# shoeffner/ann3depth

Hardware: AMD Instinct MI355X
Metric: images/sec (640x480->55x74 MSDN train step) (higher is better)
Workload: dtype f32

## Files before the change

### ann3depth_amd/csrc/fewch.hip

```cpp
#include <algorithm>

#include "a3d_internal.h"
#include "igemm.h"

namespace a3d {

enum { FEW_SRC_DZ = 0, FEW_SRC_POOLED = 1, FEW_SRC_POOLED_BF16 = 2 };
constexpr int kFewRows = 6;

struct FewchParams {
  const float* x;
  const void* dz;
  const void* pooled;
  const uint8_t* argmax;
  float* slabs;
  int n, h, w, c, R, S, stride, ho, wo, N, M, Mp, NP;
  int ldz, ld_arg;
  int rows_per_img, rows_total, splits, mgroups;
  int xpitch, rowlen, kpairs, wo_pad;
  int xvec4, dvec4;
};

typedef float f32x16 __attribute__((ext_vector_type(16)));

// ... 182 lines not shown
    A3D_STAMP(s3);
    const float* ap = xs + a_off;
    const float* bp = dzs + lh * NP + li;
    const int groups = p.kpairs >> 2;
    const bool more = row + 1 < row_hi;
    float a[2][4], b[2][4][TN];
    auto read = [&](int buf) {
#pragma unroll
      for (int u = 0; u < 4; ++u) {
        a[buf][u] = ap[u * a_step];
#pragma unroll
        for (int t = 0; t < TN; ++t) b[buf][u][t] = bp[u * 2 * NP + t * 32];
      }
      ap += 4 * a_step;
      bp += 8 * NP;
    };
    auto mul = [&](int buf) {
#pragma unroll
      for (int u = 0; u < 4; ++u)
#pragma unroll
        for (int t = 0; t < TN; ++t) acc[t] = __builtin_amdgcn_mfma_f32_32x32x2f32(a[buf][u], b[buf][u][t], acc[t], 0, 0, 0);
    };
    int g = 0;
    if (groups >= 2) {
      read(0);
      read(1);
      mul(0);
      if (more) fetch(row + 1);
      if (groups > 2) read(0);
      mul(1);
      for (g = 2; g + 2 <= groups; g += 2) {
        read(1);
        mul(0);
        if (g + 2 < groups) read(0);
        mul(1);
      }
      if (g < groups) mul(0);
      g = groups;
    } else if (more) {
      fetch(row + 1);
    }
    for (int kp = g * 4; kp < p.kpairs; ++kp) {
      const float av1 = ap[0];
#pragma unroll
      for (int t = 0; t < TN; ++t) acc[t] = __builtin_amdgcn_mfma_f32_32x32x2f32(av1, bp[t * 32], acc[t], 0, 0, 0);
      ap += a_step;
      bp += 2 * NP;
    }
#ifdef A3D_STAMPS
    A3D_STAMP(s4);
    d_ld += s_ld - s_mid; d_xw += s_mid - s1; d_bar1 += s1 - s0; d_commit += s2 - s1; d_bar2 += s3 - s2; d_mfma += s4 - s3;
#endif
  }
#ifdef A3D_STAMPS
  if (lane == 0 && blockIdx.x < 1024) {
    unsigned long long t_end;
    A3D_STAMP(t_end);
    unsigned long long* o = g_fewch_stamps + ((size_t)blockIdx.x * 4 + wv) * 8;
    o[0] = d_bar1; o[1] = d_commit; o[2] = d_bar2; o[3] = d_mfma; o[4] = (unsigned long long)(row_hi - row_lo); o[5] = d_xw; o[6] = t_end;
    o[7] = d_ld;
  }
  unsigned long long t_end2 = 0;
  A3D_STAMP(t_end2);
#endif
  float* slab = p.slabs + ((size_t)split * p.Mp + mg * 128 + wv * 32) * NP;
#pragma unroll
  for (int t = 0; t < TN; ++t)
#pragma unroll
    for (int g = 0; g < 4; ++g)
#pragma unroll
      for (int i = 0; i < 4; ++i) slab[(size_t)(8 * g + 4 * lh + i) * NP + t * 32 + li] = acc[t][4 * g + i];
#ifdef A3D_STAMPS
  asm volatile("s_waitcnt vmcnt(0)" ::: "memory");
  unsigned long long t_exit = 0;
  A3D_STAMP(t_exit);
  if (lane == 0 && blockIdx.x < 1024) {
    unsigned long long* o = g_fewch_stamps + ((size_t)blockIdx.x * 4 + wv) * 8;
    o[5] = t_exit - t_end2;
    o[6] = t_end2 - t_entry;
  }
#endif
}

__global__ __launch_bounds__(256) void fewch_reduce_kernel(const float* __restrict__ slabs, int splits, int Mp, int NP, int M, int N,
                                                           float* __restrict__ dw, float* __restrict__ db) {
  const int idx = blockIdx.x * 256 + threadIdx.x;
  if (idx >= (M + 1) * N) return;
  const int m = idx / N, n = idx - m * N;
  const float* s = slabs + (size_t)m * NP + n;
  const size_t pitch = (size_t)Mp * NP;
  float a0 = 0.f;
  int k = 0;
  for (; k + 8 <= splits; k += 8) {
    float v[8];
#pragma unroll
    for (int u = 0; u < 8; ++u) v[u] = s[(size_t)(k + u) * pitch];
#pragma unroll
    for (int u = 0; u < 8; ++u) a0 += v[u];
  }
  for (; k < splits; ++k) a0 += s[(size_t)k * pitch];
  if (m < M) dw[(size_t)m * N + n] = a0;
  else if (db) db[n] = a0;
}

struct FewchShape {
  int M, Mp, mgroups, TN, NP, rows_per_img, rows_total, splits, xpitch, wo_pad, kpairs;
  size_t lds;
};

static FewchShape fewch_shape(const a3d_conv_desc* d, bool pooled) {
  FewchShape s;
  s.M = d->r * d->s * d->c;
  s.mgroups = (s.M + 1 + 127) / 128;
  s.Mp = s.mgroups * 128;
  s.TN = (d->k + 31) / 32;
  s.NP = s.TN * 32;
  s.rows_per_img = pooled ? (d->ho / 2) * 2 : d->ho;
  s.rows_total = d->n * s.rows_per_img;
  s.wo_pad = (d->wo + 1) / 2 * 2;
  s.kpairs = s.wo_pad / 2;
  const int reach = (s.wo_pad - 1) * d->stride * d->c + d->s * d->c;
  s.xpitch = (std::max(d->w * d->c, reach) + 3) / 4 * 4;
  s.splits = std::max(1, std::min(s.rows_total / 4, tune_int("A3D_FEWCH_BLOCKS", 512) / s.mgroups));
  s.lds = (size_t)((kFewRows + 2) * s.xpitch + s.wo_pad * s.NP + 256 * 4 + s.NP + 4) * 4;
  return s;
}

bool fewch_bwdf_applicable(const a3d_conv_desc* d, bool pooled) {
  if (d->precision != A3D_PREC_F32 || d->c > 4 || d->pad_t || d->pad_l || d->ldx != d->c) return false;
  if (d->k < 33 || d->k > 96) return false;
  if (d->s * d->c < 27) return false;
  if ((d->ho - 1) * d->stride + d->r > d->h || (d->wo - 1) * d->stride + d->s > d->w) return false;
  if (pooled && (d->ho < 2 || d->wo < 2)) return false;
  if ((d->w * d->c) % 4 != 0) return false;
  if ((double)d->n * d->h * d->w * d->c * 4.0 >= 2147483647.0) return false;
  const FewchShape s = fewch_shape(d, pooled);
  if (s.rows_total < 1 || s.lds > 78 * 1024) return false;
  if (kFewRows * (d->w * d->c / 4) > kPX * 256) return false;
  if ((pooled ? d->wo / 2 : d->wo) * ((d->k + 3) / 4) > (pooled ? kPDPooled : kPDPlain) * 256) return false;
  return true;
}

bool fewch_extents_ok(const a3d_conv_desc* d, bool pooled, int ldz, int esz, int ld_arg) {
  const double pixels = pooled ? (double)d->n * (d->ho / 2) * (d->wo / 2) : (double)d->n * d->ho * d->wo;
  return pixels * ldz * esz < 2147483647.0 && (!pooled || pixels * ld_arg < 2147483647.0);
}

size_t fewch_bwdf_ws_bytes(const a3d_conv_desc* d, bool pooled) {
  const FewchShape s = fewch_shape(d, pooled);
  return (size_t)s.splits * s.Mp * s.NP * 4 + 16;
}

template <int TN, int SRC, bool VEC, int STEP>
static void fewch_launch4(const FewchParams& p, int blocks, size_t lds, hipStream_t st) {
  (void)hipFuncSetAttribute(reinterpret_cast<const void*>(&fewch_bwdf_kernel<TN, SRC, VEC, STEP>), hipFuncAttributeMaxDynamicSharedMemorySize,
                            80 * 1024);
  hipLaunchKernelGGL((fewch_bwdf_kernel<TN, SRC, VEC, STEP>), dim3(blocks), dim3(256), lds, st, p);
}
template <int TN, int SRC, bool VEC>
static void fewch_launch3(const FewchParams& p, int blocks, size_t lds, hipStream_t st) {
  const int step = p.stride * p.c;
  if (TN == 3 && step == 12) return fewch_launch4<TN, SRC, VEC, TN == 3 ? 12 : 0>(p, blocks, lds, st);
  if (TN == 2 && step == 6) return fewch_launch4<TN, SRC, VEC, TN == 2 ? 6 : 0>(p, blocks, lds, st);
  if (TN == 2 && step == 3) return fewch_launch4<TN, SRC, VEC, TN == 2 ? 3 : 0>(p, blocks, lds, st);
  fewch_launch4<TN, SRC, VEC, 0>(p, blocks, lds, st);
}
template <int TN>
static void fewch_launch(int src, const FewchParams& p, int blocks, size_t lds, hipStream_t st) {
  if (src == FEW_SRC_DZ) p.dvec4 ? fewch_launch3<TN, FEW_SRC_DZ, true>(p, blocks, lds, st) : fewch_launch3<TN, FEW_SRC_DZ, false>(p, blocks, lds, st);
  else if (src == FEW_SRC_POOLED) p.dvec4 ? fewch_launch3<TN, FEW_SRC_POOLED, true>(p, blocks, lds, st) : fewch_launch3<TN, FEW_SRC_POOLED, false>(p, blocks, lds, st);
  else p.dvec4 ? fewch_launch3<TN, FEW_SRC_POOLED_BF16, true>(p, blocks, lds, st) : fewch_launch3<TN, FEW_SRC_POOLED_BF16, false>(p, blocks, lds, st);
}

int fewch_bwd_filter(const a3d_conv_desc* d, const float* x, int src, const void* dz, int ldz, const void* pooled_act,
                     const uint8_t* argmax, int ld_arg, float* dw, float* db, void* ws, hipStream_t st) {
  const bool pooled = src != FEW_SRC_DZ;
  const FewchShape s = fewch_shape(d, pooled);
  FewchParams p{};
  p.x = x; p.dz = dz; p.pooled = pooled_act; p.argmax = argmax;
  p.slabs = reinterpret_cast<float*>((reinterpret_cast<uintptr_t>(ws) + 15) & ~(uintptr_t)15);
  p.n = d->n; p.h = d->h; p.w = d->w; p.c = d->c; p.R = d->r; p.S = d->s; p.stride = d->stride; p.ho = d->ho; p.wo = d->wo;
  p.N = d->k; p.M = s.M; p.Mp = s.Mp; p.NP = s.NP; p.ldz = ldz; p.ld_arg = ld_arg;
  p.rows_per_img = s.rows_per_img; p.rows_total = s.rows_total; p.splits = s.splits; p.mgroups = s.mgroups;
  p.xpitch = s.xpitch; p.rowlen = d->w * d->c; p.kpairs = s.kpairs; p.wo_pad = s.wo_pad;
  p.xvec4 = p.rowlen % 4 == 0 && (reinterpret_cast<uintptr_t>(x) & 15) == 0;
  p.dvec4 = pooled ? (d->k % 4 == 0 && ld_arg % 4 == 0 && (reinterpret_cast<uintptr_t>(argmax) & 3) == 0)
                   : (d->k % 4 == 0 && ldz % 4 == 0 && (reinterpret_cast<uintptr_t>(dz) & 15) == 0);
  const int blocks = s.splits * s.mgroups;
  clear_stale_error();
  if (s.TN == 3) fewch_launch<3>(src, p, blocks, s.lds, st);
  else fewch_launch<2>(src, p, blocks, s.lds, st);
  int rc = check_launch("fewch_bwd_filter");
  if (rc != A3D_OK) return rc;
  return fewch_reduce_launch(p.slabs, s.splits, s.Mp, s.NP, s.M, d->k, dw, db, st);
}

#ifdef A3D_STAMPS
extern "C" int a3d_debug_fewch_stamps(unsigned long long* out, size_t bytes) {
  (void)hipDeviceSynchronize();
  return (int)hipMemcpyFromSymbol(out, HIP_SYMBOL(g_fewch_stamps), std::min(bytes, sizeof(g_fewch_stamps)));
}
#endif

int fewch_reduce_launch(const float* slabs, int splits, int Mp, int NP, int M, int N, float* dw, float* db, hipStream_t st) {
  const int outs = (M + 1) * N;
  clear_stale_error();
  hipLaunchKernelGGL(fewch_reduce_kernel, dim3((outs + 255) / 256), dim3(256), 0, st, slabs, splits, Mp, NP, M, N, dw, db);
  return check_launch("fewch_reduce");
}

}
```

### ann3depth_amd/csrc/igemm.h

```cpp
#pragma once
#include <hip/hip_runtime.h>
#include <stdint.h>

#include <type_traits>

#include "igemm_plan.h"

namespace a3d {

#ifdef A3D_STAMPS
#define A3D_STAMP(var)                                                                         \
  do {                                                                                         \
    __builtin_amdgcn_sched_barrier(0);                                                         \
    unsigned long long t_;                                                                     \
    asm volatile("s_memtime %0\n\ts_waitcnt lgkmcnt(0)" : "=s"(t_)::"memory");                 \
    __builtin_amdgcn_sched_barrier(0);                                                         \
    var = t_;                                                                                  \
  } while (0)
#define A3D_RTSTAMP(var)                                                                       \
  do {                                                                                         \
    __builtin_amdgcn_sched_barrier(0);                                                         \
    unsigned long long t_;                                                                     \
    asm volatile("s_memrealtime %0\n\ts_waitcnt lgkmcnt(0)" : "=s"(t_)::"memory");             \
    __builtin_amdgcn_sched_barrier(0);                                                         \
// ... 333 lines not shown
  return (uint32_t)(((unsigned long long)b * total) / nblk);
}

template <int TM, int TN>
__device__ __forceinline__ void slab_store(float* slab, const f32x16 (&acc)[TM][TN], int wave, int lane) {
#pragma unroll
  for (int a = 0; a < TM; ++a)
#pragma unroll
    for (int b = 0; b < TN; ++b)
#pragma unroll
      for (int q = 0; q < 4; ++q) {
        const f32x4 v = {acc[a][b][4 * q], acc[a][b][4 * q + 1], acc[a][b][4 * q + 2], acc[a][b][4 * q + 3]};
        *reinterpret_cast<f32x4*>(slab + ((((size_t)(wave * TM + a) * TN + b) * 4 + q) * 64 + lane) * 4) = v;
      }
}
template <int TM, int TN>
__device__ __forceinline__ void slab_add(const float* slab, f32x16 (&acc)[TM][TN], int wave, int lane) {
#pragma unroll
  for (int a = 0; a < TM; ++a)
#pragma unroll
    for (int b = 0; b < TN; ++b)
#pragma unroll
      for (int q = 0; q < 4; ++q) {
        const f32x4 v = *reinterpret_cast<const f32x4*>(slab + ((((size_t)(wave * TM + a) * TN + b) * 4 + q) * 64 + lane) * 4);
        acc[a][b][4 * q] += v[0]; acc[a][b][4 * q + 1] += v[1]; acc[a][b][4 * q + 2] += v[2]; acc[a][b][4 * q + 3] += v[3];
      }
}

template <int MODE>
__device__ __forceinline__ void store_quad(const IgemmParams& p, const f32x4 q, int row0, int col, float* Cout, int ldc,
                                           bool partial) {
  if (col >= p.N) return;
  float v[4];
  size_t o[4];
  bool ok[4];
  const bool remap = !partial && MODE == MODE_BWD_D;
#pragma unroll
  for (int i = 0; i < 4; ++i) {
    const int row = row0 + i;
    v[i] = q[i];
    ok[i] = row < p.M;
    o[i] = (remap ? remap_row(ok[i] ? row : 0, p.sub_step, p.sub_ph, p.sub_pw, p.outW, p.outHW, p.div_phw, p.div_pw) : (size_t)row) *
               ldc + col;
  }
  if (!partial) {
    if (MODE == MODE_FWD) {
      const float bias = p.bias ? p.bias[col] : 0.f;
#pragma unroll
      for (int i = 0; i < 4; ++i) v[i] += bias;
      if (p.act == EPI_RELU) {
#pragma unroll
        for (int i = 0; i < 4; ++i) v[i] = fmaxf(v[i], 0.f);
      } else if (p.act == EPI_SIGMOID) {
#pragma unroll
        for (int i = 0; i < 4; ++i) v[i] = 1.f / (1.f + __expf(-v[i]));
      }
      if (p.keep) {
        uint8_t k[4];
#pragma unroll
        for (int i = 0; i < 4; ++i) k[i] = ok[i] ? p.keep[(size_t)(row0 + i) * p.N + col] : (uint8_t)0;
#pragma unroll
        for (int i = 0; i < 4; ++i) v[i] = k[i] ? v[i] * p.mask_scale : 0.f;
      }
    } else if (MODE == MODE_BWD_D) {
      if (p.mask) {
        float y[4];
#pragma unroll
        for (int i = 0; i < 4; ++i) y[i] = ok[i] ? p.mask[o[i]] : 0.f;
#pragma unroll
        for (int i = 0; i < 4; ++i) v[i] = apply_act_grad(v[i], y[i], p.mask_act, p.mask_scale);
      }
    }
  }
  if (p.c16 && !partial) {
#pragma unroll
    for (int i = 0; i < 4; ++i)
      if (ok[i]) reinterpret_cast<__bf16*>(Cout)[o[i]] = (__bf16)v[i];
  } else {
#pragma unroll
    for (int i = 0; i < 4; ++i)
      if (ok[i]) Cout[o[i]] = v[i];
  }
}
template <int MODE, int TM, int TN, int WM, int WN>
__device__ __forceinline__ void store_tile(const IgemmParams& p, const f32x16 (&acc)[TM][TN], int m0, int n0, int wm,
                                           int wn, int li, int lh, float* Cout, int ldc, bool partial) {
#pragma unroll
  for (int a = 0; a < TM; ++a)
#pragma unroll
    for (int b = 0; b < TN; ++b)
#pragma unroll
      for (int q = 0; q < 4; ++q) {
        const f32x4 v = {acc[a][b][4 * q], acc[a][b][4 * q + 1], acc[a][b][4 * q + 2], acc[a][b][4 * q + 3]};
        store_quad<MODE>(p, v, m0 + wm * WM + a * 32 + 8 * q + 4 * lh, n0 + wn * WN + b * 32 + li, Cout, ldc, partial);
      }
}

__device__ __forceinline__ __amdgpu_buffer_rsrc_t epi_rsrc(const void* base, size_t byte_off, uint32_t bytes) {
  const unsigned long long a = reinterpret_cast<unsigned long long>(base) + byte_off;
  const uint32_t lo = __builtin_amdgcn_readfirstlane((uint32_t)a), hi = __builtin_amdgcn_readfirstlane((uint32_t)(a >> 32));
  return __builtin_amdgcn_make_buffer_rsrc(reinterpret_cast<void*>(((unsigned long long)hi << 32) | lo), 0,
                                           (int)__builtin_amdgcn_readfirstlane(bytes), 0x00020000);
}
template <int MODE>
__device__ __forceinline__ bool epi_buf_ok(const IgemmParams& p, int ldc, bool partial) {
  if (ldc >= (1 << 21)) return false;
  if (partial) return true;
  if (MODE == MODE_BWD_D && p.sub_step > 1) return false;
  if (MODE == MODE_FWD && p.keep) return false;
  return true;
}
template <int MODE, int BM, int TM, int TN, int WM, int WN, bool MASK16, bool FASTEXP = true>
__device__ __forceinline__ void store_tile_buf(const IgemmParams& p, f32x16 (&acc)[TM][TN], int m0, int n0, int wm, int wn,
                                               int li, int lh, float* Cout, int ldc, bool partial, bool c16) {
  int rows_left = p.M - m0;
  rows_left = rows_left < 0 ? 0 : (rows_left > BM ? BM : rows_left);
  const uint32_t row_el = (uint32_t)((wm * WM + 4 * lh) * ldc);
  uint32_t elb[TN];
  bool okb[TN];
#pragma unroll
  for (int b = 0; b < TN; ++b) {
    const int col = n0 + wn * WN + b * 32 + li;
    okb[b] = col < p.N;
    elb[b] = row_el + (uint32_t)col;
  }
  auto row_off = [&](int a, int e) -> uint32_t { return (uint32_t)((a * 32 + 8 * (e >> 2) + (e & 3)) * ldc); };
  if (!partial) {
    if (MODE == MODE_FWD) {
      float bias[TN];
#pragma unroll
      for (int b = 0; b < TN; ++b) bias[b] = (p.bias && okb[b]) ? p.bias[n0 + wn * WN + b * 32 + li] : 0.f;
#pragma unroll
      for (int a = 0; a < TM; ++a)
#pragma unroll
        for (int b = 0; b < TN; ++b)
#pragma unroll
          for (int e = 0; e < 16; ++e) acc[a][b][e] += bias[b];
      if (p.act == EPI_RELU) {
#pragma unroll
        for (int a = 0; a < TM; ++a)
#pragma unroll
          for (int b = 0; b < TN; ++b)
#pragma unroll
            for (int e = 0; e < 16; ++e) acc[a][b][e] = fmaxf(acc[a][b][e], 0.f);
      } else if (p.act == EPI_SIGMOID) {
#pragma unroll
        for (int a = 0; a < TM; ++a)
#pragma unroll
          for (int b = 0; b < TN; ++b)
#pragma unroll
            for (int e = 0; e < 16; ++e) acc[a][b][e] = 1.f / (1.f + (FASTEXP ? __expf(-acc[a][b][e]) : expf(-acc[a][b][e])));
      }
    } else if (MODE == MODE_BWD_D) {
      if (p.mask) {
        constexpr uint32_t MSZ = MASK16 ? 2u : 4u;
        const __amdgpu_buffer_rsrc_t rsM = epi_rsrc(p.mask, (size_t)m0 * ldc * MSZ, (uint32_t)(rows_left * ldc) * MSZ);
#pragma unroll
        for (int a = 0; a < TM; ++a)
#pragma unroll
          for (int b = 0; b < TN; ++b) {
            const uint32_t vb = okb[b] ? elb[b] * MSZ : kOOB;
            float y[16];
#pragma unroll
            for (int e = 0; e < 16; ++e) {
              if constexpr (MASK16)
                y[e] = (float)__builtin_bit_cast(
// ... 488 lines not shown
        }
      }
    } else {
#pragma unroll
    for (int u = 0; u < BK / 8; ++u) {
      f32x4 af[TM], bf[TN];
      const int kk = 8 * u + 4 * lh;
#pragma unroll
      for (int a = 0; a < TM; ++a) {
        const int row = (wm * Cfg::WM + a * 32 + li) ^ (Cfg::A_SWZ ? 32 * lh : 0);
        if (MODE == MODE_BWD_F) {
#pragma unroll
          for (int j = 0; j < 4; ++j) af[a][j] = Ac[(kk + j) * Cfg::A_LD + row];
        } else {
          af[a] = *reinterpret_cast<const f32x4*>(Ac + row * Cfg::A_LD + kk);
        }
      }
#pragma unroll
      for (int b = 0; b < TN; ++b) {
        const int col = (wn * Cfg::WN + b * 32 + li) ^ (Cfg::B_SWZ ? 32 * lh : 0);
        if (MODE == MODE_BWD_D) {
          bf[b] = *reinterpret_cast<const f32x4*>(Bc + col * Cfg::B_LD + kk);
        } else {
#pragma unroll
          for (int j = 0; j < 4; ++j) bf[b][j] = Bc[(kk + j) * Cfg::B_LD + col];
        }
      }
      if (u == BK / 8 - 1) {
        A3D_STAMP(s2);
        if (more) store_tiles(cur ^ 1);
        A3D_STAMP(s3);
      }
#pragma unroll
      for (int j = 0; j < 4; ++j)
#pragma unroll
        for (int a = 0; a < TM; ++a)
#pragma unroll
          for (int b = 0; b < TN; ++b)
            acc[a][b] = __builtin_amdgcn_mfma_f32_32x32x2f32(af[a][j], bf[b][j], acc[a][b], 0, 0, 0);
    }
    }
    A3D_STAMP(s4);
    __syncthreads();
    A3D_STAMP(s5);
#ifdef A3D_STAMPS
    d01 += s1 - s0; d12 += s2 - s1; d23 += s3 - s2; d34 += s4 - s3; d45 += s5 - s4;
#endif
  };
  for (int it = 0; it < nkt; it += 2) {
    tile_body(it, std::integral_constant<int, 0>{});
    if (it + 1 < nkt) tile_body(it + 1, std::integral_constant<int, 1>{});
  }
  };
  if constexpr (MODE == MODE_BWD_F) {
    k_loop(std::false_type{});
  } else {
    if (p.uni) k_loop(std::true_type{});
    else k_loop(std::false_type{});
  }
#ifdef A3D_STAMPS
  A3D_STAMP(tend);
  A3D_RTSTAMP(rtend);
  if (p.stamps && lane == 0) {
    unsigned long long* o = p.stamps + ((size_t)bid_in * NWAVES + wave) * 16;
    o[0] = d01; o[1] = d12; o[2] = d23; o[3] = d34; o[4] = d45; o[5] = tend - tbeg; o[6] = (unsigned long long)nkt; o[7] = tp1 - t_entry; o[15] = tp2 - tp1;
    o[8] = tbeg - t_entry; o[9] = t_entry; o[10] = tend; o[12] = rtend - rtbeg; o[13] = rtbeg; o[14] = rtend;
  }
#define A3D_STAMP_EXIT()                                                                                   \
  do {                                                                                                     \
    unsigned long long t_exit_;                                                                            \
    A3D_STAMP(t_exit_);                                                                                    \
    if (p.stamps && lane == 0) p.stamps[((size_t)bid_in * NWAVES + wave) * 16 + 11] = t_exit_;              \
  } while (0)
#else
#define A3D_STAMP_EXIT() do { } while (0)
#endif

  igemm_epilogue<MODE, BM, BN, TM, TN, Cfg::WM, Cfg::WN>(p, acc, split, bid, seg, kt_begin, kt_end, nk_total, do_bias, bsum, tid, wave, lane,
                                                          m0, n0, wm, wn);
  }
  A3D_STAMP_EXIT();
}

template <int MODE, int BM, int BN, int WAVES_M, int NWAVES>
__global__ __launch_bounds__(256) void igemm_fixup_kernel(const IgemmParams p, const uint32_t nblk) {
  constexpr int WAVES_N = NWAVES / WAVES_M, WM = BM / WAVES_M, WN = BN / WAVES_N, TM = WM / 32, TN = WN / 32;
  constexpr int UNITS = NWAVES * TM * TN * 4;
  constexpr int MAXC = 1024;
  __shared__ uint32_t slots[MAXC];
  __shared__ uint32_t nslots;
  const int lane = threadIdx.x & 63;
  const int unit = (int)blockIdx.y * 4 + (int)(threadIdx.x >> 6);
  const uint32_t tile = blockIdx.x;
  const uint32_t nk = p.div_nk.d, tiles = (uint32_t)(p.tiles_m * p.tiles_n);
  if (threadIdx.x == 0) {
    uint32_t n = 0;
    const uint32_t total = tiles * nk, t0 = tile * nk, t1 = t0 + nk - 1;
    uint32_t jf = (uint32_t)(((unsigned long long)t0 * nblk) / total), jl = (uint32_t)(((unsigned long long)t1 * nblk) / total);
    while (jf + 1 < nblk && sk_first(jf + 1, nblk, total) <= t0) ++jf;
    while (jl + 1 < nblk && sk_first(jl + 1, nblk, total) <= t1) ++jl;
    for (uint32_t b = jf; b <= jl; ++b) {
      const uint32_t f = sk_first(b, nblk, total);
      if (f == sk_first(b + 1, nblk, total)) continue;
      if (n < MAXC) slots[n] = 2 * b + (f / nk == tile ? 0u : 1u);
      ++n;
    }
    nslots = n < MAXC ? n : MAXC;
  }
  __syncthreads();
  const uint32_t n = nslots;
  if (n <= 1) return;
  const int tile_m = (int)tile / p.tiles_n, tile_n = (int)tile - tile_m * p.tiles_n;
  if (unit < UNITS) {
    const size_t uoff = ((size_t)unit * 64 + lane) * 4;
    f32x4 s = {0.f, 0.f, 0.f, 0.f};
    auto slab_of = [&](uint32_t i) -> f32x4 {
      return *reinterpret_cast<const f32x4*>(p.sk_ws + (size_t)slots[i] * (size_t)(BM * BN) + uoff);
    };
    uint32_t i = 0;
    for (; i + 8 <= n; i += 8) {
      f32x4 v[8];
#pragma unroll
      for (int u = 0; u < 8; ++u) v[u] = slab_of(i + u);
#pragma unroll
      for (int u = 0; u < 8; ++u) s += v[u];
    }
    if (i + 4 <= n) {
      const f32x4 v0 = slab_of(i), v1 = slab_of(i + 1), v2 = slab_of(i + 2), v3 = slab_of(i + 3);
      s += v0; s += v1; s += v2; s += v3;
      i += 4;
    }
    for (; i < n; ++i) s += slab_of(i);
    const int q = unit & 3, ab = unit >> 2, bb = ab % TN, a = (ab / TN) % TM, wave = ab / (TN * TM);
    const int wm = wave / WAVES_N, wn = wave % WAVES_N, li = lane & 31, lh = lane >> 5;
    store_quad<MODE>(p, s, tile_m * BM + wm * WM + a * 32 + 8 * q + 4 * lh, tile_n * BN + wn * WN + bb * 32 + li, p.C,
                     p.ldc, false);
  }
  if (MODE == MODE_BWD_F && p.dbias != nullptr && tile_m == 0 && blockIdx.y == 0 && (int)threadIdx.x < BN) {
    static_assert(BN <= 256, "bias sums by the first 256 threads");
    float bsum = 0.f;
    for (uint32_t i = 0; i < n; ++i) bsum += p.sk_bias[(size_t)slots[i] * BN + threadIdx.x];
    if (tile_n * BN + (int)threadIdx.x < p.N) p.dbias[tile_n * BN + threadIdx.x] = bsum;
  }
}

template <int MODE, int BM, int BN, int WAVES_M, int NWAVES, int BKT, int AVEC, int BVEC>
__global__ __launch_bounds__(64 * NWAVES, (BKT == 16 ? 3 : 2) * NWAVES / 4) void igemm_kernel(const IgemmParams p) {
  igemm_body<MODE, BM, BN, WAVES_M, NWAVES, BKT, AVEC, BVEC>(p, gridDim.x, blockIdx.x);
}

struct IgemmMulti {
  IgemmParams p[4];
};
template <int MODE, int BM, int BN, int WAVES_M, int NWAVES, int BKT, int AVEC, int BVEC>
__global__ __launch_bounds__(64 * NWAVES, (BKT == 16 ? 3 : 2) * NWAVES / 4) void igemm_multi_kernel(const IgemmMulti ps) {
  const IgemmParams& p = ps.p[blockIdx.y];
  const uint32_t nwg = (uint32_t)(p.tiles_m * p.tiles_n * p.splitk);
  if (blockIdx.x >= nwg) return;
  igemm_body<MODE, BM, BN, WAVES_M, NWAVES, BKT, AVEC, BVEC>(p, nwg, blockIdx.x);
}

struct ReduceParams {
  const float* ws; float* C; const float* bias; const float* mask; const uint8_t* keep; float mask_scale;
  int M, N, ldc, splitk, act, mode, mask_act; size_t slab;
  int sub_step, sub_ph, sub_pw, outW, outHW; FastDiv div_phw, div_pw;
  int vec4;
  int c16;
  const float* dbias_ws; float* dbias_out;
  int dbias_splits;
  unsigned dbias_block0;
  void* C2; int ld2, step2, off2, c2_16, cols2;
  int c_cols;
  int row_rl, row_rlp;
};
__global__ __launch_bounds__(256) void splitk_reduce_kernel(const ReduceParams p);

}
```

### ann3depth_amd/csrc/igemm_host.hip

```cpp
#include <algorithm>
#include <cmath>
#include <cstdio>
#include <cstdlib>
#include <mutex>
#include <vector>

#include "a3d_internal.h"
#include "igemm.h"
#include "igemm_cfgs.h"

namespace a3d {

int launch_igemm_mode0(int cfg, int avec, int bvec, IgemmParams& p, unsigned grid, hipStream_t st);
int launch_igemm_mode1(int cfg, int avec, int bvec, IgemmParams& p, unsigned grid, hipStream_t st);
int launch_igemm_mode2(int cfg, int avec, int bvec, IgemmParams& p, unsigned grid, hipStream_t st);
int launch_igemm_bf16(int mode, int bn, bool x3, IgemmParams& p, unsigned grid, hipStream_t st);
int launch_fixup_mode0(int cfg, IgemmParams& p, unsigned tiles, unsigned nblk, hipStream_t st);
int launch_fixup_mode1(int cfg, IgemmParams& p, unsigned tiles, unsigned nblk, hipStream_t st);
int launch_fixup_mode2(int cfg, IgemmParams& p, unsigned tiles, unsigned nblk, hipStream_t st);
int launch_igemm_multi_bwd_d(int avec, int bvec, IgemmMulti& ps, unsigned grid_x, unsigned count, hipStream_t st);
int launch_igemm_bf16_multi_bwd_d(int bn, IgemmMulti& ps, unsigned grid_x, unsigned count, hipStream_t st);
int launch_igemm_ring(int mode, int cfg, IgemmParams& p, unsigned grid, hipStream_t st);

#ifdef A3D_STAMPS
static unsigned long long* g_stamps = nullptr;
static unsigned g_stamp_grid = 0;
static const size_t kStampBytes = (size_t)8 << 20;
#endif

static inline bool aligned16(const void* p) { return (reinterpret_cast<uintptr_t>(p) & 15) == 0; }


struct TimingSlot {
  hipEvent_t start, stop;
  a3d_timing_record rec;
};
static std::mutex g_timing_mu;
static bool g_timing_on = false;
static bool g_timing_only = false;
static a3d_timing_record g_timing_like{};
static std::vector<TimingSlot> g_timing;

static bool timing_wanted(const a3d_timing_record& r) {
  std::lock_guard<std::mutex> lk(g_timing_mu);
  if (!g_timing_on) return false;
  if (!g_timing_only) return true;
  const a3d_timing_record& l = g_timing_like;
  return r.mode == l.mode && r.prec == l.prec && r.bm == l.bm && r.bn == l.bn && r.waves_m == l.waves_m &&
         r.nwaves == l.nwaves && r.bk == l.bk && r.avec == l.avec && r.bvec == l.bvec && r.lds_dma == l.lds_dma;
}
static int timing_begin(TimingSlot& slot, hipStream_t st) {
  if (hipEventCreate(&slot.start) != hipSuccess || hipEventCreate(&slot.stop) != hipSuccess)
    return set_error(A3D_ELAUNCH, "timing: hipEventCreate failed");
  (void)hipEventRecord(slot.start, st);
  return A3D_OK;
}
static void timing_end(TimingSlot& slot, hipStream_t st) {
  (void)hipEventRecord(slot.stop, st);
  std::lock_guard<std::mutex> lk(g_timing_mu);
  g_timing.push_back(slot);
}
static a3d_timing_record timing_record(int mode, int prec, int bm, int bn, int waves_m, int nwaves, int bk, int avec, int bvec,
                                       int lds_dma, int m, int n, int k) {
  a3d_timing_record r{};
  r.mode = mode; r.prec = prec; r.bm = bm; r.bn = bn; r.waves_m = waves_m; r.nwaves = nwaves; r.bk = bk;
  r.avec = avec; r.bvec = bvec; r.lds_dma = lds_dma; r.splitk = 1; r.m = m; r.n = n; r.k = k; r.ms = 0.f;
  r.flops = 2.0 * m * n * k;
  return r;
}
template <typename Launch>
static int timed_launch(const a3d_timing_record& rec, hipStream_t st, Launch&& launch) {
  if (!timing_wanted(rec)) return launch();
  TimingSlot slot{};
  slot.rec = rec;
  int rc = timing_begin(slot, st);
  if (rc != A3D_OK) return rc;
  rc = launch();
  timing_end(slot, st);
  return rc;
}

template <typename V>
__device__ __forceinline__ V slab_sum(const V* ws, size_t slab, int splitk, size_t i) {
  V s = V(0.f);
  int z = 0;
  for (; z + 8 <= splitk; z += 8) {
    V t[8];
#pragma unroll
    for (int u = 0; u < 8; ++u) t[u] = ws[(size_t)(z + u) * slab + i];
#pragma unroll
    for (int u = 0; u < 8; ++u) s += t[u];
  }
  if (z + 4 <= splitk) {
    const V a = ws[(size_t)z * slab + i], b = ws[(size_t)(z + 1) * slab + i];
    const V c = ws[(size_t)(z + 2) * slab + i], d = ws[(size_t)(z + 3) * slab + i];
    s += a; s += b; s += c; s += d;
    z += 4;
  }
  for (; z < splitk; ++z) s += ws[(size_t)z * slab + i];
  return s;
}

__device__ __forceinline__ size_t unpadded_pos(size_t i, int nv, int rl, int rlp) {
  if (rlp == 0) return i;
  const size_t row = i / (size_t)nv, c = i - row * (size_t)nv;
  const size_t rr = row / (size_t)rlp, q = row - rr * (size_t)rlp;
  return q < (size_t)rl ? (rr * (size_t)rl + q) * (size_t)nv + c : SIZE_MAX;
}
template <typename V>
__device__ __forceinline__ void reduce_wide(const V* src, V* dst, size_t slab, size_t count, int splitk, size_t first, V* lds, int nv,
                                            int rl, int rlp);
__global__ __launch_bounds__(256) void splitk_reduce_kernel(const ReduceParams p) {
  const size_t total = (size_t)p.M * p.N;
  unsigned nblk = gridDim.x;
  if (p.dbias_splits > 0) {
    __shared__ float lds[256];
    if (blockIdx.x >= p.dbias_block0) {
      reduce_wide<float>(p.dbias_ws, p.dbias_out, (size_t)p.N, (size_t)p.N, p.dbias_splits, (size_t)(blockIdx.x - p.dbias_block0) * 16, lds,
                         0, 0, 0);
      return;
    }
    nblk = p.dbias_block0;
  } else if (p.dbias_out) {
    for (size_t i = (size_t)blockIdx.x * 256 + threadIdx.x; i < (size_t)p.N; i += (size_t)gridDim.x * 256)
      p.dbias_out[i] = slab_sum<float>(p.dbias_ws, (size_t)p.N, p.splitk, i);
  }
  if (p.vec4) {
    typedef float f4 __attribute__((ext_vector_type(4)));
    const size_t nv = total / 4;
    const f4* ws4 = reinterpret_cast<const f4*>(p.ws);
    const size_t slab4 = p.slab / 4;
    for (size_t i = (size_t)blockIdx.x * 256 + threadIdx.x; i < nv; i += (size_t)nblk * 256) {
      const size_t o = unpadded_pos(i, p.N / 4, p.row_rl, p.row_rlp);
      if (o != SIZE_MAX) reinterpret_cast<f4*>(p.C)[o] = slab_sum<f4>(ws4, slab4, p.splitk, i);
    }
    return;
  }
  for (size_t i = (size_t)blockIdx.x * 256 + threadIdx.x; i < total; i += (size_t)nblk * 256) {
    float s = slab_sum<float>(p.ws, p.slab, p.splitk, i);
    const int row = (int)(i / p.N), col = (int)(i - (size_t)row * p.N);
    const size_t o = remap_row(row, p.mode == MODE_BWD_D ? p.sub_step : 1, p.sub_ph, p.sub_pw, p.outW, p.outHW, p.div_phw,
                               p.div_pw) * p.ldc + col;
    if (p.mode == MODE_FWD) {
      if (p.bias) s += p.bias[col];
      if (p.act == EPI_RELU) s = fmaxf(s, 0.f);
      else if (p.act == EPI_SIGMOID) s = 1.f / (1.f + expf(-s));
      if (p.keep) s = p.keep[i] ? s * p.mask_scale : 0.f;
    } else if (p.mode == MODE_BWD_D) {
      if (p.mask) {
        const float y = p.c16 ? (float)reinterpret_cast<const __bf16*>(p.mask)[o] : p.mask[o];
        s = apply_act_grad(s, y, p.mask_act, p.mask_scale);
      }
    }
    if (p.c_cols == 0 || col < p.c_cols) {
      if (p.c16) reinterpret_cast<__bf16*>(p.C)[o] = (__bf16)s;
      else p.C[o] = s;
    }
    if (p.C2 && col < p.cols2) {
      const size_t o2 = ((size_t)row * p.ld2 + col) * p.step2 + p.off2;
      if (p.c2_16) static_cast<__bf16*>(p.C2)[o2] = (__bf16)(p.c16 ? (float)(__bf16)s : s);
      else static_cast<float*>(p.C2)[o2] = p.c16 ? (float)(__bf16)s : s;
    }
  }
}

__global__ __launch_bounds__(256) void second_output_kernel(const void* C, int c16, int M, int ldc, void* C2, int ld2, int step2, int off2,
                                                            int c2_16, int cols2) {
  const size_t total = (size_t)M * cols2;
  for (size_t i = (size_t)blockIdx.x * 256 + threadIdx.x; i < total; i += (size_t)gridDim.x * 256) {
    const int row = (int)(i / cols2), col = (int)(i - (size_t)row * cols2);
    const size_t o = (size_t)row * ldc + col;
    const float s = c16 ? (float)static_cast<const __bf16*>(C)[o] : static_cast<const float*>(C)[o];
    const size_t o2 = ((size_t)row * ld2 + col) * step2 + off2;
    if (c2_16) static_cast<__bf16*>(C2)[o2] = (__bf16)s;
    else static_cast<float*>(C2)[o2] = s;
  }
}

template <typename V>
__device__ __forceinline__ void reduce_wide(const V* src, V* dst, size_t slab, size_t count, int splitk, size_t first,
                                            V* lds, int nv, int rl, int rlp) {
  const int tid = threadIdx.x, out = tid & 15, part = tid >> 4;
// ... 1038 lines not shown
```

### ann3depth_amd/csrc/igemm_inst.h

```cpp
#include "a3d_internal.h"
#include "igemm.h"
#include "igemm_cfgs.h"
#include "igemm_glds.h"

namespace a3d {

template <int NWAVES>
constexpr size_t share_lds_bytes(size_t need) {
  constexpr size_t blocks = NWAVES >= 8 ? 1 : 8 / NWAVES;
  const size_t pad = (size_t)163840 / (blocks + 1) + 1024;
  return need > pad ? need : pad;
}

template <int BM, int BN, int WAVES_M, int NWAVES, int BK, int AVEC, int BVEC>
static int launch_one(IgemmParams& p, unsigned grid, hipStream_t st) {
  using Cfg = IgemmCfg<A3D_MODE, BM, BN, WAVES_M, NWAVES, BK, AVEC, BVEC>;
  auto kern = igemm_kernel<A3D_MODE, BM, BN, WAVES_M, NWAVES, BK, AVEC, BVEC>;
  constexpr size_t kShared = share_lds_bytes<NWAVES>(Cfg::LDS_BYTES);
  static bool attr_done = false;
  if (!attr_done) {
    hipError_t e = hipFuncSetAttribute(reinterpret_cast<const void*>(kern),
                                       hipFuncAttributeMaxDynamicSharedMemorySize, (int)kShared);
    if (e != hipSuccess) return set_error(A3D_ELAUNCH, "hipFuncSetAttribute: %s", hipGetErrorString(e));
    attr_done = true;
  }
  clear_stale_error();
  hipLaunchKernelGGL(kern, dim3(grid), dim3(Cfg::NT), p.share ? kShared : Cfg::LDS_BYTES, st, p);
  return check_launch("igemm");
}

template <int BM, int BN, int WAVES_M, int NWAVES, int BK>
static int launch_vec(int avec, int bvec, IgemmParams& p, unsigned grid, hipStream_t st) {
  if (avec == 4 && bvec == 4) return launch_one<BM, BN, WAVES_M, NWAVES, BK, 4, 4>(p, grid, st);
  if (avec == 4 && bvec == 1) return launch_one<BM, BN, WAVES_M, NWAVES, BK, 4, 1>(p, grid, st);
  if (avec == 1 && bvec == 4) return launch_one<BM, BN, WAVES_M, NWAVES, BK, 1, 4>(p, grid, st);
  if (avec == 2 && bvec == 4) return launch_one<BM, BN, WAVES_M, NWAVES, BK, 2, 4>(p, grid, st);
  if (avec == 2 && bvec == 1) return launch_one<BM, BN, WAVES_M, NWAVES, BK, 2, 1>(p, grid, st);
  return launch_one<BM, BN, WAVES_M, NWAVES, BK, 1, 1>(p, grid, st);
}

template <int BM, int BN, int WAVES_M, int NWAVES>
static int launch_glds(IgemmParams& p, unsigned grid, hipStream_t st) {
  using Cfg = GldsCfg<A3D_MODE, BM, BN, WAVES_M, NWAVES>;
  auto kern = igemm_glds_kernel<A3D_MODE, BM, BN, WAVES_M, NWAVES>;
  static bool attr_done = false;
  if (!attr_done) {
    hipError_t e = hipFuncSetAttribute(reinterpret_cast<const void*>(kern),
                                       hipFuncAttributeMaxDynamicSharedMemorySize, (int)Cfg::LDS_BYTES);
    if (e != hipSuccess) return set_error(A3D_ELAUNCH, "hipFuncSetAttribute: %s", hipGetErrorString(e));
    attr_done = true;
  }
  clear_stale_error();
  hipLaunchKernelGGL(kern, dim3(grid), dim3(Cfg::NT), Cfg::LDS_BYTES, st, p);
  return check_launch("igemm_glds");
}

template <int BM, int BN, int WAVES_M, int NWAVES>
static int launch_fixup_one(IgemmParams& p, unsigned tiles, unsigned nblk, hipStream_t st) {
  clear_stale_error();
  hipLaunchKernelGGL((igemm_fixup_kernel<A3D_MODE, BM, BN, WAVES_M, NWAVES>), dim3(tiles, (BM * BN / 256 + 3) / 4), dim3(256),
                     0, st, p, nblk);
  return check_launch("igemm_fixup");
}

#if A3D_MODE == 1
template <int AVEC, int BVEC>
static int launch_multi_one(IgemmMulti& ps, unsigned grid_x, unsigned count, hipStream_t st) {
  using Cfg = IgemmCfg<MODE_BWD_D, 64, 64, 2, 4, 32, AVEC, BVEC>;
  auto kern = igemm_multi_kernel<MODE_BWD_D, 64, 64, 2, 4, 32, AVEC, BVEC>;
  static bool attr_done = false;
  if (!attr_done) {
    hipError_t e = hipFuncSetAttribute(reinterpret_cast<const void*>(kern),
                                       hipFuncAttributeMaxDynamicSharedMemorySize, (int)Cfg::LDS_BYTES);
    if (e != hipSuccess) return set_error(A3D_ELAUNCH, "hipFuncSetAttribute: %s", hipGetErrorString(e));
    attr_done = true;
  }
  clear_stale_error();
  hipLaunchKernelGGL(kern, dim3(grid_x, count), dim3(Cfg::NT), Cfg::LDS_BYTES, st, ps);
  return check_launch("igemm_multi");
}
int launch_igemm_multi_bwd_d(int avec, int bvec, IgemmMulti& ps, unsigned grid_x, unsigned count, hipStream_t st) {
  if (avec == 4 && bvec == 4) return launch_multi_one<4, 4>(ps, grid_x, count, st);
  if (avec == 4 && bvec == 1) return launch_multi_one<4, 1>(ps, grid_x, count, st);
  if (avec == 1 && bvec == 4) return launch_multi_one<1, 4>(ps, grid_x, count, st);
  return launch_multi_one<1, 1>(ps, grid_x, count, st);
}
#endif

#define A3D_CAT_(a, b) a##b
#define A3D_CAT(a, b) A3D_CAT_(a, b)

int A3D_CAT(launch_fixup_mode, A3D_MODE)(int cfg, IgemmParams& p, unsigned tiles, unsigned nblk, hipStream_t st) {
  switch (cfg) {
#define X(i, bm, bn, wm, nw, bk, eff) \
  case i: return launch_fixup_one<bm, bn, wm, nw>(p, tiles, nblk, st);
    A3D_CFGS(X)
#undef X
  }
  return set_error(A3D_EINVAL, "igemm fixup: unknown config %d", cfg);
}

int A3D_CAT(launch_igemm_mode, A3D_MODE)(int cfg, int avec, int bvec, IgemmParams& p, unsigned grid, hipStream_t st) {
  switch (cfg) {
#define X(i, bm, bn, wm, nw, twin, eff) \
  case i:                               \
    if (avec == 4 && bvec == 4) return launch_glds<bm, bn, wm, nw>(p, grid, st); \
    cfg = twin;                    \
    break;
    A3D_GLDS_CFGS(X)
#undef X
  }
  switch (cfg) {
#define X(i, bm, bn, wm, nw, bk, eff) \
  case i: return launch_vec<bm, bn, wm, nw, bk>(avec, bvec, p, grid, st);
    A3D_CFGS(X)
#undef X
  }
  return set_error(A3D_EINVAL, "igemm: unknown config %d", cfg);
}

}
```

Baseline: 11630.

## Restructure split-K reduction kernels for wider loads and per-wave slot discovery

```diff
diff --git a/ann3depth_amd/csrc/fewch.hip b/ann3depth_amd/csrc/fewch.hip
--- a/ann3depth_amd/csrc/fewch.hip
+++ b/ann3depth_amd/csrc/fewch.hip
@@ -288,25 +288,56 @@
 #endif
 }
 
+#ifndef A3D_FIXUP_NT
+#define A3D_FIXUP_NT 1
+#endif
+constexpr int kRedSplits = 128;
 __global__ __launch_bounds__(256) void fewch_reduce_kernel(const float* __restrict__ slabs, int splits, int Mp, int NP, int M, int N,
                                                            float* __restrict__ dw, float* __restrict__ db) {
-  const int idx = blockIdx.x * 256 + threadIdx.x;
-  if (idx >= (M + 1) * N) return;
-  const int m = idx / N, n = idx - m * N;
-  const float* s = slabs + (size_t)m * NP + n;
+  typedef float f4 __attribute__((ext_vector_type(4)));
+  __shared__ f4 rows[kRedSplits][16];
+  const int tid = threadIdx.x, c4 = tid & 15, part = tid >> 4;
+  const size_t image = (size_t)(M + 1) * NP;
   const size_t pitch = (size_t)Mp * NP;
+  const size_t e4 = (size_t)blockIdx.x * 64 + (size_t)c4 * 4;
+  const size_t e = (size_t)blockIdx.x * 64 + tid;
+  const float* lds = reinterpret_cast<const float*>(&rows[0][0]);
   float a0 = 0.f;
-  int k = 0;
-  for (; k + 8 <= splits; k += 8) {
-    float v[8];
-#pragma unroll
-    for (int u = 0; u < 8; ++u) v[u] = s[(size_t)(k + u) * pitch];
-#pragma unroll
-    for (int u = 0; u < 8; ++u) a0 += v[u];
-  }
-  for (; k < splits; ++k) a0 += s[(size_t)k * pitch];
-  if (m < M) dw[(size_t)m * N + n] = a0;
-  else if (db) db[n] = a0;
+  for (int k0 = 0; k0 < splits; k0 += kRedSplits) {
+    const int cnt = min(splits - k0, kRedSplits);
+    if (e4 < image) {
+      f4 v[kRedSplits / 16];
+#pragma unroll
+      for (int j = 0; j < kRedSplits / 16; ++j)
+        if (j * 16 + part < cnt) {
+          const f4* src = reinterpret_cast<const f4*>(slabs + (size_t)(k0 + j * 16 + part) * pitch + e4);
+          v[j] = A3D_FIXUP_NT ? __builtin_nontemporal_load(src) : *src;
+        }
+#pragma unroll
+      for (int j = 0; j < kRedSplits / 16; ++j)
+        if (j * 16 + part < cnt) rows[j * 16 + part][c4] = v[j];
+    }
+    __syncthreads();
+    if (tid < 64 && e < image) {
+      int k = 0;
+      for (; k + 8 <= cnt; k += 8) {
+        float t[8];
+#pragma unroll
+        for (int u = 0; u < 8; ++u) t[u] = lds[(k + u) * 64 + tid];
+#pragma unroll
+        for (int u = 0; u < 8; ++u) a0 += t[u];
+      }
+      for (; k < cnt; ++k) a0 += lds[k * 64 + tid];
+    }
+    __syncthreads();
+  }
+  if (tid < 64 && e < image) {
+    const int m = (int)(e / NP), n = (int)(e - (size_t)m * NP);
+    if (n < N) {
+      if (m < M) dw[(size_t)m * N + n] = a0;
+      else if (db) db[n] = a0;
+    }
+  }
 }
 
 struct FewchShape {
@@ -409,9 +440,9 @@
 #endif
 
 int fewch_reduce_launch(const float* slabs, int splits, int Mp, int NP, int M, int N, float* dw, float* db, hipStream_t st) {
-  const int outs = (M + 1) * N;
+  const size_t image = (size_t)(M + 1) * NP;
   clear_stale_error();
-  hipLaunchKernelGGL(fewch_reduce_kernel, dim3((outs + 255) / 256), dim3(256), 0, st, slabs, splits, Mp, NP, M, N, dw, db);
+  hipLaunchKernelGGL(fewch_reduce_kernel, dim3((unsigned)((image + 63) / 64)), dim3(256), 0, st, slabs, splits, Mp, NP, M, N, dw, db);
   return check_launch("fewch_reduce");
 }
 
diff --git a/ann3depth_amd/csrc/igemm.h b/ann3depth_amd/csrc/igemm.h
--- a/ann3depth_amd/csrc/igemm.h
+++ b/ann3depth_amd/csrc/igemm.h
@@ -439,6 +439,81 @@
       if (ok[i]) Cout[o[i]] = v[i];
   }
 }
+template <int MODE, int U>
+__device__ __forceinline__ void store_quads(const IgemmParams& p, const f32x4 (&q)[U], const int (&row0)[U], const int (&col)[U],
+                                            float* Cout, int ldc) {
+  float v[U][4];
+  size_t o[U][4];
+  bool ok[U][4];
+#pragma unroll
+  for (int u = 0; u < U; ++u)
+#pragma unroll
+    for (int i = 0; i < 4; ++i) {
+      const int row = row0[u] + i;
+      v[u][i] = q[u][i];
+      ok[u][i] = col[u] < p.N && row < p.M;
+      o[u][i] = (MODE == MODE_BWD_D ? remap_row(ok[u][i] ? row : 0, p.sub_step, p.sub_ph, p.sub_pw, p.outW, p.outHW, p.div_phw, p.div_pw)
+                                    : (size_t)row) * ldc + col[u];
+    }
+  if (MODE == MODE_FWD) {
+    float bias[U];
+#pragma unroll
+    for (int u = 0; u < U; ++u) bias[u] = (p.bias && col[u] < p.N) ? p.bias[col[u]] : 0.f;
+    uint8_t k[U][4];
+    if (p.keep) {
+#pragma unroll
+      for (int u = 0; u < U; ++u)
+#pragma unroll
+        for (int i = 0; i < 4; ++i) k[u][i] = ok[u][i] ? p.keep[(size_t)(row0[u] + i) * p.N + col[u]] : (uint8_t)0;
+    }
+#pragma unroll
+    for (int u = 0; u < U; ++u)
+#pragma unroll
+      for (int i = 0; i < 4; ++i) v[u][i] += bias[u];
+    if (p.act == EPI_RELU) {
+#pragma unroll
+      for (int u = 0; u < U; ++u)
+#pragma unroll
+        for (int i = 0; i < 4; ++i) v[u][i] = fmaxf(v[u][i], 0.f);
+    } else if (p.act == EPI_SIGMOID) {
+#pragma unroll
+      for (int u = 0; u < U; ++u)
+#pragma unroll
+        for (int i = 0; i < 4; ++i) v[u][i] = 1.f / (1.f + __expf(-v[u][i]));
+    }
+    if (p.keep) {
+#pragma unroll
+      for (int u = 0; u < U; ++u)
+#pragma unroll
+        for (int i = 0; i < 4; ++i) v[u][i] = k[u][i] ? v[u][i] * p.mask_scale : 0.f;
+    }
+  } else if (MODE == MODE_BWD_D) {
+    if (p.mask) {
+      float y[U][4];
+#pragma unroll
+      for (int u = 0; u < U; ++u)
+#pragma unroll
+        for (int i = 0; i < 4; ++i) y[u][i] = ok[u][i] ? p.mask[o[u][i]] : 0.f;
+#pragma unroll
+      for (int u = 0; u < U; ++u)
+#pragma unroll
+        for (int i = 0; i < 4; ++i) v[u][i] = apply_act_grad(v[u][i], y[u][i], p.mask_act, p.mask_scale);
+    }
+  }
+  if (p.c16) {
+#pragma unroll
+    for (int u = 0; u < U; ++u)
+#pragma unroll
+      for (int i = 0; i < 4; ++i)
+        if (ok[u][i]) reinterpret_cast<__bf16*>(Cout)[o[u][i]] = (__bf16)v[u][i];
+  } else {
+#pragma unroll
+    for (int u = 0; u < U; ++u)
+#pragma unroll
+      for (int i = 0; i < 4; ++i)
+        if (ok[u][i]) Cout[o[u][i]] = v[u][i];
+  }
+}
 template <int MODE, int TM, int TN, int WM, int WN>
 __device__ __forceinline__ void store_tile(const IgemmParams& p, const f32x16 (&acc)[TM][TN], int m0, int n0, int wm,
                                            int wn, int li, int lh, float* Cout, int ldc, bool partial) {
@@ -1093,66 +1168,124 @@
   A3D_STAMP_EXIT();
 }
 
+#ifndef A3D_FIXUP_NT
+#define A3D_FIXUP_NT 1
+#endif
+template <int MODE>
+struct FixupShape {
+  static constexpr int U = MODE == MODE_BWD_F ? 4 : 8;
+  static constexpr int CMAX = 32 / U;
+};
 template <int MODE, int BM, int BN, int WAVES_M, int NWAVES>
 __global__ __launch_bounds__(256) void igemm_fixup_kernel(const IgemmParams p, const uint32_t nblk) {
   constexpr int WAVES_N = NWAVES / WAVES_M, WM = BM / WAVES_M, WN = BN / WAVES_N, TM = WM / 32, TN = WN / 32;
   constexpr int UNITS = NWAVES * TM * TN * 4;
-  constexpr int MAXC = 1024;
-  __shared__ uint32_t slots[MAXC];
-  __shared__ uint32_t nslots;
+  constexpr int U = FixupShape<MODE>::U, CMAX = FixupShape<MODE>::CMAX;
+  constexpr uint32_t GROUPS = UNITS / U;
+  static_assert(UNITS % U == 0 && BN <= 64 * (int)GROUPS, "unit groups; bias sums by the first BN / 64 groups");
   const int lane = threadIdx.x & 63;
-  const int unit = (int)blockIdx.y * 4 + (int)(threadIdx.x >> 6);
-  const uint32_t tile = blockIdx.x;
+  const uint32_t w = __builtin_amdgcn_readfirstlane(blockIdx.x * 4 + (threadIdx.x >> 6));
   const uint32_t nk = p.div_nk.d, tiles = (uint32_t)(p.tiles_m * p.tiles_n);
-  if (threadIdx.x == 0) {
-    uint32_t n = 0;
-    const uint32_t total = tiles * nk, t0 = tile * nk, t1 = t0 + nk - 1;
-    uint32_t jf = (uint32_t)(((unsigned long long)t0 * nblk) / total), jl = (uint32_t)(((unsigned long long)t1 * nblk) / total);
-    while (jf + 1 < nblk && sk_first(jf + 1, nblk, total) <= t0) ++jf;
-    while (jl + 1 < nblk && sk_first(jl + 1, nblk, total) <= t1) ++jl;
-    for (uint32_t b = jf; b <= jl; ++b) {
-      const uint32_t f = sk_first(b, nblk, total);
-      if (f == sk_first(b + 1, nblk, total)) continue;
-      if (n < MAXC) slots[n] = 2 * b + (f / nk == tile ? 0u : 1u);
-      ++n;
-    }
-    nslots = n < MAXC ? n : MAXC;
-  }
-  __syncthreads();
-  const uint32_t n = nslots;
+  const uint32_t tile = w / GROUPS, grp = w - tile * GROUPS;
+  if (tile >= tiles) return;
+  const uint32_t total = tiles * nk, t0 = tile * nk, t1 = t0 + nk - 1;
+  const uint32_t qt = total / nblk, rt = total - qt * nblk;
+  auto first = [&](uint32_t b) -> uint32_t { return b * qt + (b * rt) / nblk; };
+  const uint32_t j0 = tile < (1u << 21) ? (tile * nblk) / tiles : (uint32_t)(((unsigned long long)tile * nblk) / tiles);
+  auto list = [&](uint32_t jb, unsigned long long& mask, uint32_t& slot) -> bool {
+    const uint32_t b = jb + (uint32_t)lane;
+    const uint32_t f = first(min(b, nblk)), g = first(min(b + 1, nblk));
+    slot = 2 * b + (f >= t0 ? 0u : 1u);
+    mask = __ballot(b < nblk && f < g && f <= t1 && g > t0);
+    return __ballot(b >= nblk || f > t1) != 0ull;
+  };
+  unsigned long long mask0;
+  uint32_t slot0;
+  const bool last0 = list(j0, mask0, slot0);
+  uint32_t n = (uint32_t)__builtin_popcountll(mask0);
+  {
+    bool last = last0;
+    for (uint32_t jb = j0 + 64; !last; jb += 64) {
+      unsigned long long m;
+      uint32_t sl;
+      last = list(jb, m, sl);
+      n += (uint32_t)__builtin_popcountll(m);
+    }
+  }
   if (n <= 1) return;
   const int tile_m = (int)tile / p.tiles_n, tile_n = (int)tile - tile_m * p.tiles_n;
-  if (unit < UNITS) {
-    const size_t uoff = ((size_t)unit * 64 + lane) * 4;
-    f32x4 s = {0.f, 0.f, 0.f, 0.f};
-    auto slab_of = [&](uint32_t i) -> f32x4 {
-      return *reinterpret_cast<const f32x4*>(p.sk_ws + (size_t)slots[i] * (size_t)(BM * BN) + uoff);
+  const size_t uoff = ((size_t)grp * U * 64 + lane) * 4;
+  const bool do_bias = MODE == MODE_BWD_F && p.dbias != nullptr && tile_m == 0 && (int)grp * 64 < BN;
+  const int bcol = (int)grp * 64 + lane;
+  f32x4 s[U];
+#pragma unroll
+  for (int u = 0; u < U; ++u) s[u] = f32x4{0.f, 0.f, 0.f, 0.f};
+  float bsum = 0.f;
+  unsigned long long mask = mask0;
+  uint32_t slot = slot0;
+  bool last = last0;
+  for (uint32_t jb = j0;;) {
+    unsigned long long m = mask;
+    auto next_slot = [&]() -> uint32_t {
+      const int l = __builtin_ctzll(m);
+      m &= m - 1;
+      return (uint32_t)__builtin_amdgcn_readlane((int)slot, l);
     };
-    uint32_t i = 0;
-    for (; i + 8 <= n; i += 8) {
-      f32x4 v[8];
-#pragma unroll
-      for (int u = 0; u < 8; ++u) v[u] = slab_of(i + u);
-#pragma unroll
-      for (int u = 0; u < 8; ++u) s += v[u];
-    }
-    if (i + 4 <= n) {
-      const f32x4 v0 = slab_of(i), v1 = slab_of(i + 1), v2 = slab_of(i + 2), v3 = slab_of(i + 3);
-      s += v0; s += v1; s += v2; s += v3;
-      i += 4;
-    }
-    for (; i < n; ++i) s += slab_of(i);
+    auto round = [&](auto cc) {
+      constexpr int C = decltype(cc)::value;
+      f32x4 v[C][U];
+#pragma unroll
+      for (int c = 0; c < C; ++c) {
+        const f32x4* src = reinterpret_cast<const f32x4*>(p.sk_ws + (size_t)next_slot() * (size_t)(BM * BN) + uoff);
+#pragma unroll
+        for (int u = 0; u < U; ++u) v[c][u] = A3D_FIXUP_NT ? __builtin_nontemporal_load(src + u * 64) : src[u * 64];
+      }
+#pragma unroll
+      for (int c = 0; c < C; ++c)
+#pragma unroll
+        for (int u = 0; u < U; ++u) s[u] += v[c][u];
+    };
+    uint32_t cnt = (uint32_t)__builtin_popcountll(mask);
+    for (; cnt >= (uint32_t)CMAX; cnt -= CMAX) round(std::integral_constant<int, CMAX>{});
+    switch (cnt) {
+      case 1: round(std::integral_constant<int, 1>{}); break;
+      case 2: round(std::integral_constant<int, 2>{}); break;
+      case 3: round(std::integral_constant<int, 3>{}); break;
+      case 4: if constexpr (CMAX > 4) round(std::integral_constant<int, 4>{}); break;
+      case 5: if constexpr (CMAX > 5) round(std::integral_constant<int, 5>{}); break;
+      case 6: if constexpr (CMAX > 6) round(std::integral_constant<int, 6>{}); break;
+      case 7: if constexpr (CMAX > 7) round(std::integral_constant<int, 7>{}); break;
+      default: break;
+    }
+    if (do_bias && bcol < BN) {
+      m = mask;
+      for (cnt = (uint32_t)__builtin_popcountll(mask); cnt > 0;) {
+        const uint32_t c8 = cnt < 8 ? cnt : 8;
+        float bv[8];
+#pragma unroll
+        for (int c = 0; c < 8; ++c)
+          if ((uint32_t)c < c8) bv[c] = p.sk_bias[(size_t)next_slot() * BN + bcol];
+#pragma unroll
+        for (int c = 0; c < 8; ++c)
+          if ((uint32_t)c < c8) bsum += bv[c];
+        cnt -= c8;
+      }
+    }
+    if (last) break;
+    jb += 64;
+    last = list(jb, mask, slot);
+  }
+  int row0[U], col[U];
+#pragma unroll
+  for (int u = 0; u < U; ++u) {
+    const int unit = (int)grp * U + u;
     const int q = unit & 3, ab = unit >> 2, bb = ab % TN, a = (ab / TN) % TM, wave = ab / (TN * TM);
     const int wm = wave / WAVES_N, wn = wave % WAVES_N, li = lane & 31, lh = lane >> 5;
-    store_quad<MODE>(p, s, tile_m * BM + wm * WM + a * 32 + 8 * q + 4 * lh, tile_n * BN + wn * WN + bb * 32 + li, p.C,
-                     p.ldc, false);
-  }
-  if (MODE == MODE_BWD_F && p.dbias != nullptr && tile_m == 0 && blockIdx.y == 0 && (int)threadIdx.x < BN) {
-    static_assert(BN <= 256, "bias sums by the first 256 threads");
-    float bsum = 0.f;
-    for (uint32_t i = 0; i < n; ++i) bsum += p.sk_bias[(size_t)slots[i] * BN + threadIdx.x];
-    if (tile_n * BN + (int)threadIdx.x < p.N) p.dbias[tile_n * BN + threadIdx.x] = bsum;
-  }
+    row0[u] = tile_m * BM + wm * WM + a * 32 + 8 * q + 4 * lh;
+    col[u] = tile_n * BN + wn * WN + bb * 32 + li;
+  }
+  store_quads<MODE, U>(p, s, row0, col, p.C, p.ldc);
+  if (do_bias && bcol < BN && tile_n * BN + bcol < p.N) p.dbias[tile_n * BN + bcol] = bsum;
 }
 
 template <int MODE, int BM, int BN, int WAVES_M, int NWAVES, int BKT, int AVEC, int BVEC>
diff --git a/ann3depth_amd/csrc/igemm_host.hip b/ann3depth_amd/csrc/igemm_host.hip
--- a/ann3depth_amd/csrc/igemm_host.hip
+++ b/ann3depth_amd/csrc/igemm_host.hip
@@ -84,20 +84,22 @@
 __device__ __forceinline__ V slab_sum(const V* ws, size_t slab, int splitk, size_t i) {
   V s = V(0.f);
   int z = 0;
-  for (; z + 8 <= splitk; z += 8) {
-    V t[8];
+  for (; z + 16 <= splitk; z += 16) {
+    V t[16];
 #pragma unroll
-    for (int u = 0; u < 8; ++u) t[u] = ws[(size_t)(z + u) * slab + i];
+    for (int u = 0; u < 16; ++u) t[u] = ws[(size_t)(z + u) * slab + i];
 #pragma unroll
-    for (int u = 0; u < 8; ++u) s += t[u];
-  }
-  if (z + 4 <= splitk) {
-    const V a = ws[(size_t)z * slab + i], b = ws[(size_t)(z + 1) * slab + i];
-    const V c = ws[(size_t)(z + 2) * slab + i], d = ws[(size_t)(z + 3) * slab + i];
-    s += a; s += b; s += c; s += d;
-    z += 4;
-  }
-  for (; z < splitk; ++z) s += ws[(size_t)z * slab + i];
+    for (int u = 0; u < 16; ++u) s += t[u];
+  }
+  if (z < splitk) {
+    V t[15];
+#pragma unroll
+    for (int u = 0; u < 15; ++u)
+      if (z + u < splitk) t[u] = ws[(size_t)(z + u) * slab + i];
+#pragma unroll
+    for (int u = 0; u < 15; ++u)
+      if (z + u < splitk) s += t[u];
+  }
   return s;
 }
 
diff --git a/ann3depth_amd/csrc/igemm_inst.h b/ann3depth_amd/csrc/igemm_inst.h
--- a/ann3depth_amd/csrc/igemm_inst.h
+++ b/ann3depth_amd/csrc/igemm_inst.h
@@ -57,8 +57,11 @@
 
 template <int BM, int BN, int WAVES_M, int NWAVES>
 static int launch_fixup_one(IgemmParams& p, unsigned tiles, unsigned nblk, hipStream_t st) {
+  constexpr unsigned kWavesPerTile = BM * BN / 256 / FixupShape<A3D_MODE>::U;
+  if (nblk > 1024 || tiles > 0xffffffffu / kWavesPerTile)
+    return set_error(A3D_EINVAL, "igemm fixup: %u blocks, %u tiles", nblk, tiles);
   clear_stale_error();
-  hipLaunchKernelGGL((igemm_fixup_kernel<A3D_MODE, BM, BN, WAVES_M, NWAVES>), dim3(tiles, (BM * BN / 256 + 3) / 4), dim3(256),
+  hipLaunchKernelGGL((igemm_fixup_kernel<A3D_MODE, BM, BN, WAVES_M, NWAVES>), dim3((tiles * kWavesPerTile + 3) / 4), dim3(256),
                      0, st, p, nblk);
   return check_launch("igemm_fixup");
 }
```

Result: no change. 11570 (-0.5%).
